# limix/CellRegMap

Hardware: AMD Instinct MI355X
Metric: variant-tests/sec (interaction test) (higher is better)
Workload: dtype f64

## Files before the change

### cellregmap_amd/csrc/api_core.hip

```cpp
#include <dlfcn.h>

#include <algorithm>
#include <atomic>
#include <cstdarg>
#include <mutex>

#include <map>

#include "crm_internal.h"
#include "eigh.h"

namespace crm {

static thread_local std::string g_error;

void set_error(const char* fmt, ...) {
    char buf[1024];
    va_list ap;
    va_start(ap, fmt);
    vsnprintf(buf, sizeof buf, fmt, ap);
    va_end(ap);
    g_error = buf;
}

// ... 131 lines not shown
    if (ptr) check_redzone(ptr, bytes);
    if (ptr) (void)hipFree(ptr);
    g_live_bytes -= (long)bytes;
    ptr = nullptr;
    bytes = 0;
    serial = 0;
}

int upload_padded(hipStream_t st, double* dst, long ld_dst, long rows_pad, const double* src,
                  long ld_src, long rows, long cols) {
    CRM_HIP(hipMemsetAsync(dst, 0, sizeof(double) * rows_pad * ld_dst, st));
    if (rows > 0 && cols > 0)
        CRM_HIP(hipMemcpy2DAsync(dst, ld_dst * sizeof(double), src, ld_src * sizeof(double),
                                 cols * sizeof(double), rows, hipMemcpyHostToDevice, st));
    return CRM_OK;
}

}

using namespace crm;

extern "C" {

const char* crm_last_error(void) { return last_error_text(); }
const char* crm_version(void) { return "0.6.0"; }

int crm_ctx_create(int device, crm_ctx** out) {
    return crm::guarded("crm_ctx_create", [&]() -> int {
    if (!out) return CRM_ERR_ARG;
    *out = nullptr;
    int count = 0;
    CRM_HIP(hipGetDeviceCount(&count));
    if (device < 0 || device >= count) {
        set_error("crm_ctx_create: device %d not present (%d visible)", device, count);
        return CRM_ERR_ARG;
    }
    CRM_HIP(hipSetDevice(device));
    crm_ctx* c = new crm_ctx();
    c->device = device;
    if (const char* e = getenv("CRM_KIN_ROUTE")) c->kin_route = std::max(0, std::min(2, atoi(e)));
    CRM_HIP(hipStreamCreateWithFlags(&c->stream, hipStreamNonBlocking));
    CRM_HIP(hipStreamCreateWithFlags(&c->upload_stream, hipStreamNonBlocking));
    CRM_HIP(hipEventCreate(&c->ev0));
    CRM_HIP(hipEventCreate(&c->ev1));
    int prio_least = 0, prio_greatest = 0;
    CRM_HIP(hipDeviceGetStreamPriorityRange(&prio_least, &prio_greatest));
    CRM_HIP(hipStreamCreateWithPriority(&c->side_stream, hipStreamNonBlocking, prio_least));
    for (hipEvent_t* e : {&c->ev_fork, &c->ev_side, &c->ev_main, &c->ev_fits}) CRM_HIP(hipEventCreateWithFlags(e, hipEventDisableTiming));
    {
        std::lock_guard<std::mutex> lock(g_ctx_mutex);
        g_contexts.push_back(c);
    }
    *out = c;
    return CRM_OK;
    });
}

int crm_ctx_trim(crm_ctx* c) {
    return crm::guarded_on("crm_ctx_trim", c, [&]() -> int {
    if (!c) return CRM_ERR_ARG;
    CRM_HIP(hipSetDevice(c->device));
    CRM_HIP(hipStreamSynchronize(c->stream));
    if (c->side_stream) CRM_HIP(hipStreamSynchronize(c->side_stream));
    std::lock_guard<std::mutex> lock(g_ctx_mutex);
    (void)trim_context(c);
    return CRM_OK;
    });
}

void crm_ctx_destroy(crm_ctx* c) {
    try {
    if (!c) return;
    (void)hipSetDevice(c->device);
    (void)hipStreamSynchronize(c->stream);
    if (c->side_stream) (void)hipStreamSynchronize(c->side_stream);
    {
        std::lock_guard<std::mutex> lock(g_ctx_mutex);
        g_contexts.erase(std::remove(g_contexts.begin(), g_contexts.end(), c), g_contexts.end());
        delete c->eigh_ws;
        c->eigh_ws = nullptr;
    }
    c->replay_clear();
    for (auto* b : c->all_bufs()) b->release();
    for (auto& e : c->timed) {
        (void)hipEventDestroy(e.first);
        (void)hipEventDestroy(e.second);
    }
    (void)hipEventDestroy(c->ev0);
    (void)hipEventDestroy(c->ev1);
    for (hipEvent_t e : {c->ev_fork, c->ev_side, c->ev_main, c->ev_fits})
        if (e) (void)hipEventDestroy(e);
    if (c->side_stream) (void)hipStreamDestroy(c->side_stream);
    (void)hipStreamDestroy(c->stream);
    if (c->upload_stream) (void)hipStreamDestroy(c->upload_stream);
    if (c->sync_timeouts_host) (void)hipHostFree(c->sync_timeouts_host);
    delete c;
    } catch (...) {
    }
}

int crm_ctx_synchronize(crm_ctx* c) {
    return crm::guarded_on("crm_ctx_synchronize", c, [&]() -> int {
    if (!c) return CRM_ERR_ARG;
    CRM_HIP(hipSetDevice(c->device));
    CRM_HIP(hipStreamSynchronize(c->stream));
    if (c->side_stream) CRM_HIP(hipStreamSynchronize(c->side_stream));
    return CRM_OK;
    });
}

int crm_set_block_variants(crm_ctx* c, int variants) {
    return crm::guarded_on("crm_set_block_variants", c, [&]() -> int {
    if (!c || variants < 0) return CRM_ERR_ARG;
    c->block_variants = variants == 0 ? 0 : (int)round_up(variants, 128);
    return CRM_OK;
    });
}

int crm_set_null_fit_polish(crm_ctx* c, int on) {
    return crm::guarded_on("crm_set_null_fit_polish", c, [&]() -> int {
    if (!c) return CRM_ERR_ARG;
    c->polish = on != 0;
    return CRM_OK;
    });
}

int crm_set_progress_callback(crm_ctx* c, void (*callback)(long, long, void*), void* user) {
    return crm::guarded_on("crm_set_progress_callback", c, [&]() -> int {
    if (!c) return CRM_ERR_ARG;
    if (callback) c->progress[std::this_thread::get_id()] = crm_ctx::Progress{callback, user};
    else c->progress.erase(std::this_thread::get_id());
    return CRM_OK;
    });
}

int crm_set_fast_rotation(crm_ctx* c, int on) {
    return crm::guarded_on("crm_set_fast_rotation", c, [&]() -> int {
    if (!c) return CRM_ERR_ARG;
    c->fast_T = on != 0;
    return CRM_OK;
    });
}

extern "C++" {
namespace crm {
namespace {
struct FormSlot { const char* name; int value; bool set; };
FormSlot g_forms[] = {{"gram_staged", 0, false}, {"kr_no_tail", 0, false}, {"nullfit_per_wave", 0, false}, {"kin_fold", 0, false},
                      {"eigh_one_stage", 0, false}, {"nullfit_exact", 0, false}, {"donor_pairs", 0, false},
                      {"pairs_without_kinship_term", 0, false}, {"flat_kappa_milli", 0, false}, {"chase_abort", 0, false}, {"nullfit_one_per_wave", 0, false},
                      {"kin_diag", 0, false}, {"donor_pairs_rotate", 0, false}, {"rho0_positions", 0, false},
                      {"rotation_tails", 0, false}, {"woodbury_ytY", 0, false},
                      {"wb_block_order", 0, false}, {"block_fused", 0, false}, {"wb_gram_fused", 0, false},
                      {"gram_strips", 0, false}, {"side_stream", 0, false}, {"wb_gram_spread", 0, false}};
std::mutex g_forms_mu;
}
int form(const char* name, int otherwise) {
    std::lock_guard<std::mutex> lock(g_forms_mu);
    for (const FormSlot& f : g_forms)
        if (strcmp(f.name, name) == 0) return f.set ? f.value : otherwise;
    return otherwise;
}
}
}

int crm_test_set_form(const char* name, int value, int reset) {
    return crm::guarded("crm_test_set_form", [&]() -> int {
    if (!name) return CRM_ERR_ARG;
    std::lock_guard<std::mutex> lock(crm::g_forms_mu);
    for (crm::FormSlot& f : crm::g_forms)
        if (strcmp(f.name, name) == 0) {
            f.value = value;
            f.set = reset == 0;
            return CRM_OK;
        }
    crm::set_error("crm_test_set_form: no kernel form is called '%s'", name);
    return CRM_ERR_ARG;
    });
}

long crm_test_tail_launches(const crm_ctx* ctx) { return ctx ? ctx->tail_launches : -1; }

long crm_test_spectrum_tail_launches(const crm_ctx* ctx) { return ctx ? ctx->spectrum_tail_launches : -1; }

long crm_test_dense_repeats(const crm_ctx* ctx) { return ctx ? ctx->dense_repeats : -1; }

long crm_test_donor_pair_blocks(const crm_ctx* ctx) { return ctx ? ctx->donor_pair_blocks : -1; }

int crm_test_gram_dma_launches(const crm_ctx* ctx, long* launches) {
    return crm::guarded("crm_test_gram_dma_launches", [&]() -> int {
    if (!ctx || !launches) return CRM_ERR_ARG;
    *launches = ctx->gram_dma_launches;
    return CRM_OK;
    });
}
int crm_test_unrelated_donor_blocks(const crm_ctx* ctx, long* blocks) {
    return crm::guarded("crm_test_unrelated_donor_blocks", [&]() -> int {
    if (!ctx || !blocks) return CRM_ERR_ARG;
    *blocks = ctx->unrelated_donor_blocks;
    return CRM_OK;
    });
}

int crm_test_fused_blocks(const crm_ctx* ctx, long* blocks) {
    return crm::guarded("crm_test_fused_blocks", [&]() -> int {
    if (!ctx || !blocks) return CRM_ERR_ARG;
    *blocks = ctx->fused_blocks;
    return CRM_OK;
    });
}

int crm_test_wb_gram_fused_blocks(const crm_ctx* ctx, long* blocks) {
    return crm::guarded("crm_test_wb_gram_fused_blocks", [&]() -> int {
    if (!ctx || !blocks) return CRM_ERR_ARG;
    *blocks = ctx->wb_gram_fused_blocks;
    return CRM_OK;
    });
}

int crm_test_side_stream_blocks(const crm_ctx* ctx, long* blocks) {
    return crm::guarded("crm_test_side_stream_blocks", [&]() -> int {
    if (!ctx || !blocks) return CRM_ERR_ARG;
    *blocks = ctx->side_stream_blocks;
    return CRM_OK;
    });
}

int crm_test_rho0_position_blocks(const crm_ctx* ctx, long* blocks) {
    return crm::guarded("crm_test_rho0_position_blocks", [&]() -> int {
    if (!ctx || !blocks) return CRM_ERR_ARG;
    *blocks = ctx->rho0_position_blocks;
    return CRM_OK;
    });
}
int crm_test_rotation_tail_launches(const crm_ctx* ctx, long* launches) {
    return crm::guarded("crm_test_rotation_tail_launches", [&]() -> int {
    if (!ctx || !launches) return CRM_ERR_ARG;
    *launches = ctx->rotation_tail_launches;
    return CRM_OK;
    });
}

long crm_test_tests_without_pair(const crm_ctx* ctx) { return ctx ? ctx->tests_without_pair : -1; }

int crm_test_set_shared_h(crm_ctx* ctx, int mode) {
    return crm::guarded_on("crm_test_set_shared_h", ctx, [&]() -> int {
    if (!ctx) return CRM_ERR_ARG;
    ctx->tune.shared_h = mode < 0 ? -1 : (mode > 0 ? 1 : 0);
    return CRM_OK;
    });
}

int crm_kernel_timer_reset(crm_ctx* c) {
    return crm::guarded_on("crm_kernel_timer_reset", c, [&]() -> int {
    if (!c) return CRM_ERR_ARG;
    CRM_HIP(hipSetDevice(c->device));
    CRM_HIP(hipStreamSynchronize(c->stream));
    c->timed_used = 0;
    c->kr_flops = 0.0;
    c->timing = true;
    return CRM_OK;
    });
}

int crm_kernel_timer_stop(crm_ctx* c) {
    return crm::guarded_on("crm_kernel_timer_stop", c, [&]() -> int {
    if (!c) return CRM_ERR_ARG;
    c->timing = false;
    return CRM_OK;
    });
}

int crm_kernel_timer_read(crm_ctx* c, double* kr_ms, long* kr_launches, double* kr_flops,
                          double* total_ms) {
    return crm::guarded_on("crm_kernel_timer_read", c, [&]() -> int {
    if (!c) return CRM_ERR_ARG;
    CRM_HIP(hipSetDevice(c->device));
    CRM_HIP(hipStreamSynchronize(c->stream));
    double ms = 0.0;
    for (size_t i = 0; i < c->timed_used; i++) {
        float t = 0.f;
        CRM_HIP(hipEventElapsedTime(&t, c->timed[i].first, c->timed[i].second));
        ms += t;
    }
    if (kr_ms) *kr_ms = ms;
    if (kr_launches) *kr_launches = (long)c->timed_used;
    if (kr_flops) *kr_flops = c->kr_flops;
    if (total_ms) *total_ms = 0.0;
    return CRM_OK;
    });
}

int crm_test_set_contraction(crm_ctx* c, int tile_width, int lds_dma) {
    return crm::guarded_on("crm_test_set_contraction", c, [&]() -> int {
    if (!c || (tile_width != 0 && tile_width != 64 && tile_width != 128 && tile_width != 160)) return CRM_ERR_ARG;
    c->tune.bn = tile_width;
    c->tune.glds = lds_dma ? 1 : 0;
    return CRM_OK;
    });
}

long crm_test_sync_fallbacks(const crm_ctx* c) { return c ? c->sync_fallbacks : -1; }
long crm_test_overruns(void) { return crm::overruns_detected(); }
long crm_test_live_device_bytes(void) { return crm::live_device_bytes(); }

int crm_test_set_kinship_route(crm_ctx* c, int on) {
    return crm::guarded_on("crm_test_set_kinship_route", c, [&]() -> int {
// ... 254 lines not shown
```

### cellregmap_amd/csrc/nullfit.hip

```cpp
#include "crm_internal.h"
#include "delta_search.h"
#include "wave_ops.h"
#include <type_traits>

namespace crm {

namespace {

template <int N, int FROM>
__device__ inline void butterfly_sums(double (&v)[N]) {
    double t[N];
    if constexpr (FROM >= 32) {
#pragma unroll
        for (int i = 0; i < N; i++) t[i] = __shfl_xor(v[i], 32, 64);
#pragma unroll
        for (int i = 0; i < N; i++) v[i] += t[i];
#pragma unroll
        for (int i = 0; i < N; i++) t[i] = lane_xor_swizzle(v[i], 16);
#pragma unroll
        for (int i = 0; i < N; i++) v[i] += t[i];
    }
#pragma unroll
    for (int i = 0; i < N; i++) t[i] = lane_xor_swizzle(v[i], 8);
#pragma unroll
    for (int i = 0; i < N; i++) v[i] += t[i];
#pragma unroll
    for (int i = 0; i < N; i++) t[i] = lane_xor_swizzle(v[i], 4);
#pragma unroll
    for (int i = 0; i < N; i++) v[i] += t[i];
#pragma unroll
    for (int i = 0; i < N; i++) t[i] = lane_xor_quad(v[i], 2);
#pragma unroll
    for (int i = 0; i < N; i++) v[i] += t[i];
#pragma unroll
    for (int i = 0; i < N; i++) t[i] = lane_xor_quad(v[i], 1);
#pragma unroll
    for (int i = 0; i < N; i++) v[i] += t[i];
}

__device__ inline double fast_rcp(double D) {
    double x = __builtin_amdgcn_rcp(D);
    double e = fma(-D, x, 1.0);
    x = fma(x, e, x);
    e = fma(-D, x, 1.0);
    return fma(x, e, x);
}

struct LogProduct {
    double mant = 1.0;
    int expo = 0;
    __device__ inline void mul(double D) {
        mant *= __builtin_amdgcn_frexp_mant(D);
        expo += __builtin_amdgcn_frexp_exp(D);
    }
    __device__ inline void renorm() {
        expo += __builtin_amdgcn_frexp_exp(mant);
        mant = __builtin_amdgcn_frexp_mant(mant);
    }
    __device__ inline double log_value() const { return log(mant) + (double)expo * 0.6931471805599453; }
};

__host__ __device__ constexpr int pair_index(int u, int v, int U) {
    return u * U - u * (u - 1) / 2 + (v - u);
}

template <int P>
__device__ inline bool cholesky(double (&A)[P][P], double& logdet) {
    logdet = 0.0;
#pragma unroll
    for (int j = 0; j < P; j++) {
        double d = A[j][j];
#pragma unroll
        for (int k = 0; k < j; k++) d -= A[j][k] * A[j][k];
        if (!(d > 0.0)) return false;
        const double l = sqrt(d);
        A[j][j] = l;
        logdet += 2.0 * log(l);
#pragma unroll
        for (int i = j + 1; i < P; i++) {
            double s = A[i][j];
#pragma unroll
            for (int k = 0; k < j; k++) s -= A[i][k] * A[j][k];
            A[i][j] = s / l;
        }
    }
    return true;
}

template <int P>
__device__ inline bool cholesky_pivots(double (&A)[P][P], double (&piv)[P]) {
#pragma unroll
    for (int j = 0; j < P; j++) {
        double d = A[j][j];
#pragma unroll
        for (int k = 0; k < j; k++) d -= A[j][k] * A[j][k];
        if (!(d > 0.0)) return false;
        const double l = sqrt(d);
        A[j][j] = l;
        piv[j] = l;
#pragma unroll
        for (int i = j + 1; i < P; i++) {
            double s = A[i][j];
#pragma unroll
            for (int k = 0; k < j; k++) s -= A[i][k] * A[j][k];
            A[i][j] = s / l;
        }
    }
    return true;
}

template <int P>
__device__ inline void cholesky_solve(const double (&L)[P][P], double (&b)[P]) {
#pragma unroll
    for (int i = 0; i < P; i++) {
        double s = b[i];
#pragma unroll
        for (int k = 0; k < i; k++) s -= L[i][k] * b[k];
        b[i] = s / L[i][i];
    }
#pragma unroll
    for (int i = P - 1; i >= 0; i--) {
        double s = b[i];
#pragma unroll
        for (int k = i + 1; k < P; k++) s -= L[k][i] * b[k];
        b[i] = s / L[i][i];
    }
}

template <int U>
__device__ __noinline__ double objective_noise_bound(const double (&bb)[U], const double (&sd)[U], const double (&pl)[U * (U + 1) / 2],
                                                     double inv_d, double rss, double df, double lsum, double n_minus_r, double log_delta,
                                                     double n, double log_s, double logdetXX, double logdetH, double p_eff) {
    double mag = 0.0;
#pragma unroll
    for (int u = 0; u < U; u++)
#pragma unroll
        for (int v = u; v < U; v++) {
            const double spec = sqrt(fabs(sd[u] * sd[v]));
            const double m_uv = spec + pl[pair_index(u, v, U)] * inv_d;
            mag += (u == v ? 1.0 : 2.0) * bb[u] * bb[v] * m_uv;
        }
    const double logs = fabs(lsum) + fabs(n_minus_r) * fabs(log_delta) + n * fabs(log_s) + df * (LOG2PI + 1.0) + fabs(logdetXX) +
                        fabs(logdetH) + p_eff * fabs(log_s);
    return 0.5 * (df * mag / fabs(rss) + logs);
}

template <int C, bool SH, bool EX, bool TR, int G = 1>
__device__ __forceinline__ void nullfit_fit(const NullFitArgs& a, const int b, const int w, const int lane,
                                            const double* sW, const double* sy, const double* sS, const int sld) {
    static_assert(G == 1 || (G == 4 && C == 1 && !EX), "four fits per wavefront: one covariate column, default arithmetic");
    const int sub = G == 1 ? lane : (lane & 15);
    constexpr int P = C + 1;
    constexpr int U = C + 2;
    constexpr int NP = U * (U + 1) / 2;
    const NullFitRho R = a.rho[w];
    const double* __restrict__ tg = R.T + (long)b * R.ldT;
    const int r = R.r;
    const double n = (double)a.n;

    double uv[NP];
#pragma unroll
    for (int i = 0; i < C; i++) {
#pragma unroll
        for (int j = i; j < C; j++) uv[pair_index(i, j, U)] = a.WW[i * C + j];
        uv[pair_index(i, C, U)] = a.gW[(long)b * a.ld_gW + i];
        uv[pair_index(i, C + 1, U)] = a.Wy[i];
    }
    uv[pair_index(C, C, U)] = a.gg[b];
    uv[pair_index(C, C + 1, U)] = a.gy[b];
    uv[pair_index(C + 1, C + 1, U)] = a.yy;

    bool use_g = true;
    double logdetXX = 0.0;
    {
        double A[P][P];
#pragma unroll
        for (int i = 0; i < P; i++)
#pragma unroll
            for (int j = 0; j <= i; j++) A[i][j] = uv[pair_index(j, i, U)];
        double ld = 0.0;
        bool ok = true;
#pragma unroll
        for (int j = 0; j < P; j++) {
            double d = A[j][j];
#pragma unroll
            for (int k = 0; k < j; k++) d -= A[j][k] * A[j][k];
            if (j == P - 1) {
                if (a.g_drop ? a.g_drop[b] != 0 : !(d > 1e-12 * A[j][j])) {
                    use_g = false;
                    break;
                }
                if (!(d > 0.0)) {
                    ok = false;
                    break;
                }
            } else if (!(d > 0.0)) {
                ok = false;
                break;
            }
            const double l = sqrt(d);
            A[j][j] = l;
            ld += 2.0 * log(l);
#pragma unroll
            for (int i = j + 1; i < P; i++) {
                double s = A[i][j];
#pragma unroll
                for (int k = 0; k < j; k++) s -= A[i][k] * A[j][k];
                A[i][j] = s / l;
            }
        }
        logdetXX = ok ? ld : NAN;
    }
    const double p_eff = use_g ? (double)P : (double)C;
    const double df = a.restricted ? n - p_eff : n;

    auto spectrum_pass = [&](double delta, bool weighted, double (&S)[NP], double& lsum,
                             bool grad, double (&S2)[NP], double& lsum2) {
#pragma unroll
        for (int i = 0; i < NP; i++) { S[i] = 0.0; S2[i] = 0.0; }
        lsum = 0.0;
        lsum2 = 0.0;
        LogProduct lp;
        int trips = 0;
        const double omd = 1.0 - delta;
        constexpr int UNR = C <= 2 ? 4 : 2;
        auto trip = [&](const int j0, auto full_tag) {
            constexpr bool FULL = decltype(full_tag)::value;
            double t[UNR][U], s0[UNR];
            bool ok[UNR];
#pragma unroll
            for (int q = 0; q < UNR; q++) {
                const int j = j0 + 64 * q;
                ok[q] = FULL || j < r;
                const int jj = ok[q] ? j : r - 1;
#pragma unroll
                for (int i = 0; i < C; i++) t[q][i] = SH ? sW[i * sld + jj] : R.tW[(long)i * R.ldW + jj];
                t[q][C] = tg[jj];
                t[q][C + 1] = SH ? sy[jj] : R.ty[jj];
                s0[q] = weighted ? (SH ? sS[jj] : R.S0[jj]) : 0.0;
            }
#pragma unroll
            for (int q = 0; q < UNR; q++) {
                double wgt = ok[q] ? 1.0 : 0.0, wgt2 = 0.0;
                if (weighted) {
                    const double D = ok[q] ? omd * s0[q] + delta : 1.0;
                    const double inv = EX ? 1.0 / D : fast_rcp(D);
                    wgt = ok[q] ? inv : 0.0;
                    if (EX) lsum += log(D);
                    else lp.mul(D);
                    if (grad) {
                        const double oms = 1.0 - s0[q];
                        lsum2 += ok[q] ? oms * inv : 0.0;
                        wgt2 = ok[q] ? oms * inv * inv : 0.0;
                    }
                }
#pragma unroll
                for (int u = 0; u < U; u++) {
                    const double tw = t[q][u] * wgt;
                    const double tw2 = t[q][u] * wgt2;
#pragma unroll
                    for (int v = u; v < U; v++) {
                        S[pair_index(u, v, U)] += tw * t[q][v];
                        if (grad) S2[pair_index(u, v, U)] += tw2 * t[q][v];
                    }
                }
            }
        };
        for (int j0 = lane; j0 < r; j0 += 64 * UNR) {
            if (j0 - lane + 64 * UNR - 1 < r) trip(j0, std::true_type{});
            else trip(j0, std::false_type{});
            if (!EX && weighted && (++trips & 127) == 0) lp.renorm();
        }
        {
            double red[NP + 1];
#pragma unroll
            for (int i = 0; i < NP; i++) red[i] = S[i];
            red[NP] = weighted ? (EX ? lsum : lp.log_value()) : 0.0;
            butterfly_sums<NP + 1, 32>(red);
#pragma unroll
            for (int i = 0; i < NP; i++) S[i] = red[i];
            if (weighted) lsum = red[NP];
        }
        if (grad) {
            double red[NP + 1];
#pragma unroll
            for (int i = 0; i < NP; i++) red[i] = S2[i];
            red[NP] = lsum2;
            butterfly_sums<NP + 1, 32>(red);
#pragma unroll
            for (int i = 0; i < NP; i++) S2[i] = red[i];
            lsum2 = red[NP];
        }
    };

    auto spectrum_pass4 = [&](double delta, bool weighted, double (&S)[NP], double& lsum) {
        double Sq[4][NP];
        LogProduct lpq[4];
#pragma unroll
        for (int q = 0; q < 4; q++)
#pragma unroll
            for (int i = 0; i < NP; i++) Sq[q][i] = 0.0;
        const double omd = 1.0 - delta;
        int trips[4];
#pragma unroll
        for (int q = 0; q < 4; q++) trips[q] = sub + 16 * q < r ? (r - (sub + 16 * q) + 255) / 256 : 0;
        const int t_all = (r + 255) / 256;
        for (int t = 0; t < t_all; t++) {
            const bool full = 256 * t + 255 < r;
#pragma unroll
            for (int q = 0; q < 4; q++) {
                if (!full && t >= trips[q]) continue;
                double tv[4][U], s0[4];
                bool ok[4];
#pragma unroll
                for (int k = 0; k < 4; k++) {
                    const int j = sub + 16 * q + 64 * (4 * t + k);
                    ok[k] = full || j < r;
                    const int jj = ok[k] ? j : r - 1;
#pragma unroll
                    for (int i = 0; i < C; i++) tv[k][i] = SH ? sW[i * sld + jj] : R.tW[(long)i * R.ldW + jj];
                    tv[k][C] = tg[jj];
                    tv[k][C + 1] = SH ? sy[jj] : R.ty[jj];
                    s0[k] = weighted ? (SH ? sS[jj] : R.S0[jj]) : 0.0;
                }
#pragma unroll
                for (int k = 0; k < 4; k++) {
                    double wgt = ok[k] ? 1.0 : 0.0;
                    if (weighted) {
                        const double D = ok[k] ? omd * s0[k] + delta : 1.0;
                        const double inv = fast_rcp(D);
                        wgt = ok[k] ? inv : 0.0;
                        lpq[q].mul(D);
                    }
#pragma unroll
                    for (int u = 0; u < U; u++) {
                        const double tw = tv[k][u] * wgt;
#pragma unroll
                        for (int v = u; v < U; v++) Sq[q][pair_index(u, v, U)] += tw * tv[k][v];
                    }
                }
                if (weighted && ((t + 1) & 127) == 0) lpq[q].renorm();
            }
        }
        double red[NP + 1];
#pragma unroll
        for (int i = 0; i < NP; i++) red[i] = (Sq[0][i] + Sq[2][i]) + (Sq[1][i] + Sq[3][i]);
        red[NP] = weighted ? (lpq[0].log_value() + lpq[2].log_value()) + (lpq[1].log_value() + lpq[3].log_value()) : 0.0;
        butterfly_sums<NP + 1, 8>(red);
#pragma unroll
        for (int i = 0; i < NP; i++) S[i] = red[i];
        lsum = weighted ? red[NP] : 0.0;
    };

    double tt[NP];
    {
        double dummy, dummy2, unused[NP];
        if constexpr (G == 1) spectrum_pass(1.0, false, tt, dummy, false, unused, dummy2);
        else spectrum_pass4(1.0, false, tt, dummy);
    }

    double cur_delta = 0.5, cur_scale = 1.0, cur_lml = -INFINITY;
    int nfev = 0;
    double memo_f[2] = {0.0, 0.0}, memo_scale[2] = {0.0, 0.0}, memo_lml[2] = {0.0, 0.0}, memo_noise[2] = {NAN, NAN};
    bool memo_set[2] = {false, false};
    bool last_clamped = false;
    bool want_noise = false;
    double cur_noise = NAN;
    auto f = [&](double x) -> double {
        nfev++;
        const double delta = logistic_clamped(x);
        const int clamp = delta == 1.0 - EPS_TINY ? 1 : (delta == EPS_TINY ? 0 : -1);
        last_clamped = clamp >= 0;
        if (clamp >= 0 && memo_set[clamp]) {
            cur_delta = delta;
            cur_scale = memo_scale[clamp];
            cur_lml = memo_lml[clamp];
            cur_noise = memo_noise[clamp];
            return memo_f[clamp];
        }
        auto remember = [&](double value) -> double {
            if (clamp >= 0) {
                memo_set[clamp] = true;
                memo_f[clamp] = value;
                memo_scale[clamp] = cur_scale;
                memo_lml[clamp] = cur_lml;
                memo_noise[clamp] = cur_noise;
            }
            return value;
        };
        double S[NP], lsum;
        if constexpr (G == 1) {
            double unused[NP], unused2;
            spectrum_pass(delta, true, S, lsum, false, unused, unused2);
        } else {
            spectrum_pass4(delta, true, S, lsum);
        }
        const double inv_d = 1.0 / delta;
        double K[NP];
#pragma unroll
        for (int i = 0; i < NP; i++) K[i] = S[i] + (uv[i] - tt[i]) * inv_d;
        double A[P][P], rhs[P], xky[P];
#pragma unroll
        for (int i = 0; i < P; i++) {
#pragma unroll
            for (int j = 0; j <= i; j++) A[i][j] = K[pair_index(j, i, U)];
            rhs[i] = K[pair_index(i, C + 1, U)];
        }
        if (!use_g) {
#pragma unroll
            for (int j = 0; j < C; j++) A[C][j] = 0.0;
            A[C][C] = 1.0;
            rhs[C] = 0.0;
        }
#pragma unroll
        for (int i = 0; i < P; i++) xky[i] = rhs[i];
        double piv[P];
        double val;
        if (!cholesky_pivots<P>(A, piv)) {
            cur_delta = delta;
            cur_scale = NAN;
            cur_lml = NAN;
            return remember(INFINITY);
        }
        cholesky_solve<P>(A, rhs);
        double rss = K[pair_index(C + 1, C + 1, U)];
#pragma unroll
        for (int i = 0; i < P; i++) rss -= xky[i] * rhs[i];
        const double s = fmax(rss / df, EPS_SMALL);
        double larg = 1.0;
        larg = sub == 0 ? delta : larg;
#pragma unroll
        for (int j = 0; j < P; j++) larg = sub == 1 + j ? piv[j] : larg;
        larg = sub == P + 1 ? s : larg;
        const double lres = log(larg);
        auto from_sub = [&](int k) -> double {
            if constexpr (G == 1) return read_lane(lres, k);
            else return __shfl(lres, (lane & 48) + k, 64);
        };
        const double log_delta = from_sub(0), log_s = from_sub(P + 1);
        double logdetH = 0.0;
#pragma unroll
        for (int j = 0; j < P; j++) logdetH += 2.0 * from_sub(1 + j);
        const double logdetK = lsum + (n - (double)r) * log_delta;
        val = -0.5 * (df * LOG2PI + df + n * log_s + logdetK);
        if (a.restricted) val += 0.5 * (logdetXX - (logdetH - p_eff * log_s));
        cur_delta = delta;
        cur_scale = s;
        cur_lml = val;
        if constexpr (TR) {
            if (want_noise || clamp >= 0) {
                double bb[U], sd[U], pl[NP];
#pragma unroll
                for (int i = 0; i < P; i++) bb[i] = fabs(rhs[i]);
                bb[P] = 1.0;
#pragma unroll
                for (int u = 0; u < U; u++) sd[u] = S[pair_index(u, u, U)];
#pragma unroll
                for (int i = 0; i < NP; i++) pl[i] = fabs(uv[i]) + fabs(tt[i]);
                cur_noise = objective_noise_bound<U>(bb, sd, pl, inv_d, rss, df, lsum, (n - (double)r), log_delta, n, log_s, logdetXX,
                                                     logdetH, p_eff);
            }
        }
        return remember(-val);
    };

    auto g = [&](double x) -> double {
        const double delta = logistic_clamped(x);
        if (delta <= EPS_TINY || delta >= 1.0 - EPS_TINY) return 0.0;
        double S[NP], S2[NP], lsum, lsum2;
        spectrum_pass(delta, true, S, lsum, true, S2, lsum2);
        const double inv_d = 1.0 / delta, inv_d2 = inv_d * inv_d;
        double K[NP], dK[NP];
#pragma unroll
        for (int i = 0; i < NP; i++) {
            const double cpl = uv[i] - tt[i];
            K[i] = S[i] + cpl * inv_d;
            dK[i] = -S2[i] - cpl * inv_d2;
        }
        const double dlogdet = lsum2 + (n - (double)r) * inv_d;
        double A[P][P], dA[P][P], b[P], db[P], beta[P];
#pragma unroll
        for (int i = 0; i < P; i++) {
#pragma unroll
            for (int j = 0; j < P; j++) {
                const int pi = i <= j ? pair_index(i, j, U) : pair_index(j, i, U);
                A[i][j] = K[pi];
                dA[i][j] = dK[pi];
            }
            b[i] = K[pair_index(i, C + 1, U)];
            db[i] = dK[pair_index(i, C + 1, U)];
        }
        if (!use_g) {
#pragma unroll
            for (int j = 0; j < P; j++) {
                A[C][j] = 0.0; A[j][C] = 0.0;
                dA[C][j] = 0.0; dA[j][C] = 0.0;
            }
            A[C][C] = 1.0;
            b[C] = 0.0;
            db[C] = 0.0;
        }
        double ld;
        if (!cholesky<P>(A, ld)) return NAN;
#pragma unroll
        for (int i = 0; i < P; i++) beta[i] = b[i];
        cholesky_solve<P>(A, beta);
        double Rv = K[pair_index(C + 1, C + 1, U)];
        double dR = dK[pair_index(C + 1, C + 1, U)];
#pragma unroll
        for (int i = 0; i < P; i++) {
            Rv -= b[i] * beta[i];
            dR -= 2.0 * db[i] * beta[i];
#pragma unroll
            for (int j = 0; j < P; j++) dR += beta[i] * dA[i][j] * beta[j];
        }
        double d = df * dR / Rv + dlogdet;
        if (a.restricted) {
            double tr = 0.0;
#pragma unroll
            for (int j = 0; j < P; j++) {
                double col[P];
#pragma unroll
                for (int i = 0; i < P; i++) col[i] = dA[i][j];
                cholesky_solve<P>(A, col);
                tr += col[j];
            }
            d += tr;
        }
        return 0.5 * d * delta * (1.0 - delta);
    };

    if (a.probe) {
        (void)f(a.probe_x);
        if (sub == 0) {
            NullFitTrial t;
            t.lml = cur_lml; t.delta = cur_delta; t.scale = cur_scale; t.use_g = use_g ? 1 : 0; t.nfev = nfev;
            t.margin = NAN; t.noise = NAN; t.curv = NAN;
            a.trial[(long)b * a.nrho + w] = t;
        }
        return;
    }
    {
        struct Objective {
            decltype(f)& fn;
            const bool& at_clamp;
            __device__ inline double operator()(double x) { return fn(x); }
            __device__ inline bool clamped() const { return at_clamp; }
        } objective{f, last_clamped};
        BrentTrace trace;
        double bf0;
        double bx0 = brent_search<TR>(objective, trace, bf0);
        if constexpr (G == 1) if (a.polish) {
            const double xs = bx0, fs = bf0;
            double xa = xs, ga = g(xa);
            if (isfinite(ga) && ga != 0.0) {
                double xb = ga > 0.0 ? xa - 1e-4 : xa + 1e-4;
                double gb = g(xb);
                bool reject = false;
                for (int it = 0; it < 8; it++) {
                    if (!isfinite(gb) || gb == ga) break;
                    const double xn = xb - gb * (xb - xa) / (gb - ga);
                    if (!isfinite(xn) || fabs(xn - xs) > 1e-2) { reject = true; break; }
                    const double step = fabs(xn - xb);
                    xa = xb; ga = gb;
                    xb = xn;
                    gb = g(xb);
                    if (gb == 0.0 || step <= 1e-12 * (1.0 + fabs(xn))) break;
                }
                if (!reject && isfinite(gb)) {
                    const double fb = f(xb);
                    if (fb <= fs + 1e-9 * fabs(fs)) bx0 = xb;
                }
            }
        }
        double f_up = NAN, f_dn = NAN;
        if constexpr (TR) {
            const double tolx = 1e-6 * fabs(bx0) + 1e-6;
            f_up = f(bx0 + tolx);
            f_dn = f(bx0 - tolx);
        }
        want_noise = true;
        const double f_stop = f(bx0);
        if (sub == 0) {
            NullFitTrial t;
            t.lml = cur_lml;
            t.delta = cur_delta;
            t.scale = cur_scale;
            t.use_g = use_g ? 1 : 0;
            t.nfev = nfev;
            if constexpr (TR) {
                t.margin = fmin(trace.cmp, trace.sign);
                t.curv = 0.5 * (f_up + f_dn) - f_stop;
                t.noise = cur_noise;
            } else {
                (void)f_stop;
                t.margin = NAN; t.curv = NAN; t.noise = NAN;
            }
            a.trial[(long)b * a.nrho + w] = t;
        }
    }
}

template <int C, bool EX, bool TR>
#ifdef CRM_NULLFIT_WAVES
__attribute__((amdgpu_waves_per_eu(CRM_NULLFIT_WAVES, CRM_NULLFIT_WAVES)))
#endif
__global__ __launch_bounds__(64) void nullfit_kernel(NullFitArgs a) {
    nullfit_fit<C, false, EX, TR, 1>(a, (int)blockIdx.x, (int)blockIdx.y, (int)threadIdx.x, nullptr, nullptr, nullptr, 0);
}

constexpr int nf_shared_waves(int G) { return G == 1 ? 12 : 8; }
template <int C, bool EX, bool TR, int G>
__global__ __launch_bounds__(64 * nf_shared_waves(G)) void nullfit_shared_kernel(NullFitArgs a, int variants, int sld,
                                                                             unsigned* __restrict__ queue) {
    extern __shared__ double nf_sm[];
    __shared__ int any_left;
    double* const sW = nf_sm;
    double* const sy = nf_sm + C * sld;
    double* const sS = sy + sld;
    const int tid = threadIdx.x, lane = tid & 63;
    const int w0 = (int)(blockIdx.x % (unsigned)a.nrho);
    for (int pass = 0; pass < a.nrho; pass++) {
        const int w = (w0 + pass) % a.nrho;
        if (tid == 0)
            any_left = __hip_atomic_load(&queue[w], __ATOMIC_RELAXED, __HIP_MEMORY_SCOPE_AGENT) < (unsigned)variants;
        __syncthreads();
        const bool any = any_left != 0;
        __syncthreads();
        if (!any) continue;
        const NullFitRho R = a.rho[w];
        for (int j = tid; j < R.r; j += 64 * nf_shared_waves(G)) {
#pragma unroll
            for (int i = 0; i < C; i++) sW[i * sld + j] = R.tW[(long)i * R.ldW + j];
            sy[j] = R.ty[j];
            sS[j] = R.S0[j];
        }
        __syncthreads();
        for (;;) {
            const unsigned ticket = __hip_atomic_fetch_add(&queue[w], lane == 0 ? (unsigned)G : 0u, __ATOMIC_RELAXED,
                                                           __HIP_MEMORY_SCOPE_AGENT);
            const unsigned b0 = (unsigned)__builtin_amdgcn_readfirstlane((int)ticket);
            if (b0 >= (unsigned)variants) break;
            if constexpr (G == 1) {
                nullfit_fit<C, true, EX, TR, 1>(a, (int)b0, w, lane, sW, sy, sS, sld);
            } else {
                const unsigned b = b0 + (unsigned)(lane >> 4);
                if (b < (unsigned)variants) nullfit_fit<C, true, EX, TR, G>(a, (int)b, w, lane, sW, sy, sS, sld);
            }
        }
        __syncthreads();
    }
}

__global__ void select_rho_kernel(const NullFitTrial* __restrict__ trial, int nrho, int variants,
                                  NullFitOut* __restrict__ out) {
    const int b = blockIdx.x * blockDim.x + threadIdx.x;
    if (b >= variants) return;
    double best = -INFINITY;
    int bi = -1;
    bool fitted = true;
    for (int i = 0; i < nrho; i++) {
        const NullFitTrial t = trial[(long)b * nrho + i];
        if (t.nfev <= 0) fitted = false;
        if (t.lml > best) {
            best = t.lml;
            bi = i;
        }
    }
    NullFitOut o;
    o.use_g = trial[(long)b * nrho].use_g;
    o.decision = NAN; o.rho_decision = NAN; o.margin = NAN; o.noise = NAN; o.gap = NAN; o.curv = NAN;
    if (!fitted) {
        o.rho_index = -1;
        o.lml = NAN; o.delta = NAN; o.scale = NAN; o.v0 = NAN; o.v1 = NAN;
    } else if (bi < 0) {
        o.rho_index = 0;
        o.lml = NAN; o.delta = NAN; o.scale = NAN; o.v0 = NAN; o.v1 = NAN;
    } else {
        const NullFitTrial t = trial[(long)b * nrho + bi];
        o.rho_index = bi;
        o.lml = best;
        o.delta = t.delta;
        o.scale = t.scale;
        o.v0 = t.scale * (1.0 - t.delta);
        o.v1 = t.scale * t.delta;
        constexpr double ROUNDING = 1.1102230246251565e-16;
        o.margin = t.margin;
        o.noise = t.noise;
        o.curv = t.curv;
        o.decision = t.margin / (ROUNDING * t.noise);
        double gap = INFINITY, rdec = INFINITY;
        for (int i = 0; i < nrho; i++) {
            if (i == bi) continue;
            const NullFitTrial q = trial[(long)b * nrho + i];
            const double g = best - q.lml;
            gap = fmin(gap, g);
            rdec = fmin(rdec, g / (ROUNDING * (t.noise + q.noise)));
        }
        o.gap = gap;
        o.rho_decision = rdec;
    }
    out[b] = o;
}

}

template <int C>
static void launch_c(hipStream_t st, const NullFitArgs& a, int variants) {
    if (a.exact) hipLaunchKernelGGL((nullfit_kernel<C, true, false>), dim3(variants, a.nrho), dim3(64), 0, st, a);
    else if (a.track) hipLaunchKernelGGL((nullfit_kernel<C, false, true>), dim3(variants, a.nrho), dim3(64), 0, st, a);
    else hipLaunchKernelGGL((nullfit_kernel<C, false, false>), dim3(variants, a.nrho), dim3(64), 0, st, a);
}

int launch_nullfit(hipStream_t st, const NullFitArgs& a, int variants, bool force_wide, unsigned* queue) {
    if (variants <= 0) return CRM_OK;
    if (a.nrho < 1 || a.nrho > CRM_MAX_RHO) {
        set_error("null fit: %d grid points (supported 1..%d)", a.nrho, CRM_MAX_RHO);
        return CRM_ERR_UNSUPPORTED;
    }
    CRM_HIP(hipMemsetAsync(a.trial, 0xFF, sizeof(NullFitTrial) * (size_t)variants * a.nrho, st));
    int rmax = 1;
    for (int i = 0; i < a.nrho; i++) rmax = std::max(rmax, a.rho[i].r);
    const int sld = (rmax + 63) / 64 * 64;
    const size_t shared_lds = sizeof(double) * 3 * (size_t)sld;
    if (queue && !force_wide && a.c == 1 && variants >= 1024 && shared_lds <= 144 * 1024 && !form("nullfit_per_wave", 0)) {
        int cus = 256, dev = 0;
        CRM_HIP(hipGetDevice(&dev));
        CRM_HIP(hipDeviceGetAttribute(&cus, hipDeviceAttributeMultiprocessorCount, dev));
        CRM_HIP(hipMemsetAsync(queue, 0, sizeof(unsigned) * CRM_MAX_RHO, st));
        const bool four = !a.exact && !a.polish && rmax <= 2048 && !form("nullfit_one_per_wave", 0);
#define CRM_NF_SHARED(EXv, TRv, Gv)                                                                                        \
    do {                                                                                                                   \
        const void* fn = reinterpret_cast<const void*>(&nullfit_shared_kernel<1, EXv, TRv, Gv>);                           \
        if (shared_lds > 60 * 1024)                                                                                        \
            CRM_HIP(hipFuncSetAttribute(fn, hipFuncAttributeMaxDynamicSharedMemorySize, (int)shared_lds));                 \
        hipLaunchKernelGGL((nullfit_shared_kernel<1, EXv, TRv, Gv>), dim3(cus), dim3(64 * nf_shared_waves(Gv)), shared_lds, st, a, \
                           variants, sld, queue);                                                                          \
    } while (0)
        if (a.exact) CRM_NF_SHARED(true, false, 1);
        else if (a.track && four) CRM_NF_SHARED(false, true, 4);
        else if (a.track) CRM_NF_SHARED(false, true, 1);
        else if (four) CRM_NF_SHARED(false, false, 4);
        else CRM_NF_SHARED(false, false, 1);
#undef CRM_NF_SHARED
    } else if (a.c > CRM_MAX_COV_WIDE) {
        CRM_TRY(launch_nullfit_xwide(st, a, variants));
    } else if (force_wide || a.c > CRM_MAX_COV) {
        CRM_TRY(launch_nullfit_wide(st, a, variants));
    } else
    switch (a.c) {
        case 1: launch_c<1>(st, a, variants); break;
        case 2: launch_c<2>(st, a, variants); break;
        case 3: launch_c<3>(st, a, variants); break;
        case 4: launch_c<4>(st, a, variants); break;
        case 5: launch_c<5>(st, a, variants); break;
        case 6: launch_c<6>(st, a, variants); break;
        case 7: launch_c<7>(st, a, variants); break;
        case 8: launch_c<8>(st, a, variants); break;
        default:
            set_error("null fit: %d covariate columns (supported 1..%d)", a.c, CRM_MAX_COV);
            return CRM_ERR_UNSUPPORTED;
    }
    CRM_HIP(hipGetLastError());
    hipLaunchKernelGGL(select_rho_kernel, dim3((variants + 127) / 128), dim3(128), 0, st, a.trial, a.nrho,
                       variants, a.out);
    CRM_HIP(hipGetLastError());
    return CRM_OK;
}

}
```

Baseline: 85190.

## Share variant-independent spectrum sums across null fits and reuse the opening evaluations

In the shared-LDS null-fit kernel, the variant-independent weighted Gram sums of covariates and phenotype are computed once per rho grid point for delta=1 and the two opening deltas and stored in LDS. Each variant then runs one fused pass that computes only its genotype cross terms for all three deltas. The opening objective evaluations at x=0 and x=1 are served from a per-wave memo, and the final objective evaluation is skipped when the best point was already evaluated. This trades extra LDS, register pressure and a serial per-block precompute for fewer per-variant spectrum passes.

Result: no change. 86020, median of 6 (+1.0%).

```diff
diff --git a/cellregmap_amd/csrc/api_core.hip b/cellregmap_amd/csrc/api_core.hip
--- a/cellregmap_amd/csrc/api_core.hip
+++ b/cellregmap_amd/csrc/api_core.hip
@@ -307,7 +307,8 @@
                       {"kin_diag", 0, false}, {"donor_pairs_rotate", 0, false}, {"rho0_positions", 0, false},
                       {"rotation_tails", 0, false}, {"woodbury_ytY", 0, false},
                       {"wb_block_order", 0, false}, {"block_fused", 0, false}, {"wb_gram_fused", 0, false},
-                      {"gram_strips", 0, false}, {"side_stream", 0, false}, {"wb_gram_spread", 0, false}};
+                      {"gram_strips", 0, false}, {"side_stream", 0, false}, {"wb_gram_spread", 0, false},
+                      {"nullfit_opening", 0, false}};
 std::mutex g_forms_mu;
 }
 int form(const char* name, int otherwise) {
diff --git a/cellregmap_amd/csrc/nullfit.hip b/cellregmap_amd/csrc/nullfit.hip
--- a/cellregmap_amd/csrc/nullfit.hip
+++ b/cellregmap_amd/csrc/nullfit.hip
@@ -64,6 +64,9 @@
     return u * U - u * (u - 1) / 2 + (v - u);
 }
 
+constexpr int nf_grid_sums(int C) { return (C + 1) * (C + 2) / 2; }
+constexpr int NF_MEMO = 10;
+
 template <int P>
 __device__ inline bool cholesky(double (&A)[P][P], double& logdet) {
     logdet = 0.0;
@@ -145,9 +148,97 @@
     return 0.5 * (df * mag / fabs(rss) + logs);
 }
 
+template <int C, bool GP>
+__device__ __forceinline__ void opening_pass(const double* tg, const double* sW, const double* sy, const double* sS, const int sld,
+                                             const int r, const int lane, const double d0, const double d1,
+                                             double (&Sk)[3][GP ? (C + 1) * (C + 2) / 2 : C + 2], double (&lsum)[3]) {
+    constexpr int V = C + 1;
+    constexpr int NS = GP ? V * (V + 1) / 2 : C + 2;
+    constexpr int UNR = C <= 2 ? 4 : 2;
+#pragma unroll
+    for (int k = 0; k < 3; k++)
+#pragma unroll
+        for (int i = 0; i < NS; i++) Sk[k][i] = 0.0;
+    LogProduct lp[2];
+    int trips = 0;
+    const double omd0 = 1.0 - d0, omd1 = 1.0 - d1;
+    auto trip = [&](const int j0, auto full_tag) {
+        constexpr bool FULL = decltype(full_tag)::value;
+        double t[UNR][V], g[UNR], s0[UNR];
+        bool ok[UNR];
+#pragma unroll
+        for (int q = 0; q < UNR; q++) {
+            const int j = j0 + 64 * q;
+            ok[q] = FULL || j < r;
+            const int jj = ok[q] ? j : r - 1;
+#pragma unroll
+            for (int i = 0; i < C; i++) t[q][i] = sW[i * sld + jj];
+            t[q][C] = sy[jj];
+            g[q] = GP ? 0.0 : tg[jj];
+            s0[q] = sS[jj];
+        }
+#pragma unroll
+        for (int q = 0; q < UNR; q++) {
+            const double D0 = ok[q] ? fma(omd0, s0[q], d0) : 1.0;
+            const double D1 = ok[q] ? fma(omd1, s0[q], d1) : 1.0;
+            const double inv0 = fast_rcp(D0), inv1 = fast_rcp(D1);
+            const double wgt[3] = {ok[q] ? 1.0 : 0.0, ok[q] ? inv0 : 0.0, ok[q] ? inv1 : 0.0};
+            if constexpr (GP) {
+                lp[0].mul(D0);
+                lp[1].mul(D1);
+            }
+#pragma unroll
+            for (int k = 0; k < 3; k++) {
+                if constexpr (GP) {
+                    int i = 0;
+#pragma unroll
+                    for (int u = 0; u < V; u++) {
+                        const double tw = t[q][u] * wgt[k];
+#pragma unroll
+                        for (int v = u; v < V; v++, i++) Sk[k][i] = fma(tw, t[q][v], Sk[k][i]);
+                    }
+                } else {
+#pragma unroll
+                    for (int i = 0; i < C; i++) Sk[k][i] = fma(t[q][i] * wgt[k], g[q], Sk[k][i]);
+                    const double gw = g[q] * wgt[k];
+                    Sk[k][C] = fma(gw, g[q], Sk[k][C]);
+                    Sk[k][C + 1] = fma(gw, t[q][C], Sk[k][C + 1]);
+                }
+            }
+        }
+    };
+    for (int j0 = lane; j0 < r; j0 += 64 * UNR) {
+        if (j0 - lane + 64 * UNR - 1 < r) trip(j0, std::true_type{});
+        else trip(j0, std::false_type{});
+        if (GP && (++trips & 127) == 0) {
+            lp[0].renorm();
+            lp[1].renorm();
+        }
+    }
+    constexpr int NR = 3 * NS + (GP ? 2 : 0);
+    double red[NR];
+#pragma unroll
+    for (int k = 0; k < 3; k++)
+#pragma unroll
+        for (int i = 0; i < NS; i++) red[k * NS + i] = Sk[k][i];
+    if constexpr (GP) {
+        red[3 * NS] = lp[0].log_value();
+        red[3 * NS + 1] = lp[1].log_value();
+    }
+    butterfly_sums<NR, 32>(red);
+#pragma unroll
+    for (int k = 0; k < 3; k++)
+#pragma unroll
+        for (int i = 0; i < NS; i++) Sk[k][i] = red[k * NS + i];
+    lsum[0] = 0.0;
+    lsum[1] = GP ? red[NR - 2] : 0.0;
+    lsum[2] = GP ? red[NR - 1] : 0.0;
+}
+
 template <int C, bool SH, bool EX, bool TR, int G = 1>
 __device__ __forceinline__ void nullfit_fit(const NullFitArgs& a, const int b, const int w, const int lane,
-                                            const double* sW, const double* sy, const double* sS, const int sld) {
+                                            const double* sW, const double* sy, const double* sS, const int sld,
+                                            const bool opening, const double* sc, double* memo) {
     static_assert(G == 1 || (G == 4 && C == 1 && !EX), "four fits per wavefront: one covariate column, default arithmetic");
     const int sub = G == 1 ? lane : (lane & 15);
     constexpr int P = C + 1;
@@ -352,20 +443,135 @@
         lsum = weighted ? red[NP] : 0.0;
     };
 
-    double tt[NP];
-    {
-        double dummy, dummy2, unused[NP];
-        if constexpr (G == 1) spectrum_pass(1.0, false, tt, dummy, false, unused, dummy2);
-        else spectrum_pass4(1.0, false, tt, dummy);
-    }
-
     double cur_delta = 0.5, cur_scale = 1.0, cur_lml = -INFINITY;
     int nfev = 0;
+    double tt[NP];
+    constexpr bool KEEP_BEST = !TR && !EX;
+    bool opened = false;
+    if constexpr (KEEP_BEST) {
+        memo[0] = NAN;
+        memo[3] = INFINITY;
+    }
+    auto note_best = [&](double x, double value) {
+        if constexpr (KEEP_BEST) {
+            if (value <= memo[3]) {
+                memo[0] = x;
+                memo[1] = cur_scale;
+                memo[2] = cur_lml;
+                memo[3] = value;
+            }
+        }
+    };
     double memo_f[2] = {0.0, 0.0}, memo_scale[2] = {0.0, 0.0}, memo_lml[2] = {0.0, 0.0}, memo_noise[2] = {NAN, NAN};
     bool memo_set[2] = {false, false};
     bool last_clamped = false;
     bool want_noise = false;
     double cur_noise = NAN;
+    auto objective_of_sums = [&](const double delta, const double (&S)[NP], const double lsum, const bool noise_now) -> double {
+        const double inv_d = 1.0 / delta;
+        double K[NP];
+#pragma unroll
+        for (int i = 0; i < NP; i++) K[i] = S[i] + (uv[i] - tt[i]) * inv_d;
+        double A[P][P], rhs[P], xky[P];
+#pragma unroll
+        for (int i = 0; i < P; i++) {
+#pragma unroll
+            for (int j = 0; j <= i; j++) A[i][j] = K[pair_index(j, i, U)];
+            rhs[i] = K[pair_index(i, C + 1, U)];
+        }
+        if (!use_g) {
+#pragma unroll
+            for (int j = 0; j < C; j++) A[C][j] = 0.0;
+            A[C][C] = 1.0;
+            rhs[C] = 0.0;
+        }
+#pragma unroll
+        for (int i = 0; i < P; i++) xky[i] = rhs[i];
+        double piv[P];
+        double val;
+        if (!cholesky_pivots<P>(A, piv)) {
+            cur_delta = delta;
+            cur_scale = NAN;
+            cur_lml = NAN;
+            return INFINITY;
+        }
+        cholesky_solve<P>(A, rhs);
+        double rss = K[pair_index(C + 1, C + 1, U)];
+#pragma unroll
+        for (int i = 0; i < P; i++) rss -= xky[i] * rhs[i];
+        const double s = fmax(rss / df, EPS_SMALL);
+        double larg = 1.0;
+        larg = sub == 0 ? delta : larg;
+#pragma unroll
+        for (int j = 0; j < P; j++) larg = sub == 1 + j ? piv[j] : larg;
+        larg = sub == P + 1 ? s : larg;
+        const double lres = log(larg);
+        auto from_sub = [&](int k) -> double {
+            if constexpr (G == 1) return read_lane(lres, k);
+            else return __shfl(lres, (lane & 48) + k, 64);
+        };
+        const double log_delta = from_sub(0), log_s = from_sub(P + 1);
+        double logdetH = 0.0;
+#pragma unroll
+        for (int j = 0; j < P; j++) logdetH += 2.0 * from_sub(1 + j);
+        const double logdetK = lsum + (n - (double)r) * log_delta;
+        val = -0.5 * (df * LOG2PI + df + n * log_s + logdetK);
+        if (a.restricted) val += 0.5 * (logdetXX - (logdetH - p_eff * log_s));
+        cur_delta = delta;
+        cur_scale = s;
+        cur_lml = val;
+        if constexpr (TR) {
+            if (noise_now) {
+                double bb[U], sd[U], pl[NP];
+#pragma unroll
+                for (int i = 0; i < P; i++) bb[i] = fabs(rhs[i]);
+                bb[P] = 1.0;
+#pragma unroll
+                for (int u = 0; u < U; u++) sd[u] = S[pair_index(u, u, U)];
+#pragma unroll
+                for (int i = 0; i < NP; i++) pl[i] = fabs(uv[i]) + fabs(tt[i]);
+                cur_noise = objective_noise_bound<U>(bb, sd, pl, inv_d, rss, df, lsum, (n - (double)r), log_delta, n, log_s, logdetXX,
+                                                     logdetH, p_eff);
+            }
+        }
+        return -val;
+    };
+
+    if constexpr (SH && G == 1 && !EX) {
+        if (opening && !a.probe) {
+            constexpr int SCS = nf_grid_sums(C) + 2;
+            const double d0 = sc[SCS + SCS - 1], d1 = sc[2 * SCS + SCS - 1];
+            double Sg[3][U], unused[3];
+            opening_pass<C, false>(tg, sW, sy, sS, sld, r, lane, d0, d1, Sg, unused);
+            auto sums_of = [&](const int k, double (&S)[NP]) {
+#pragma unroll
+                for (int u = 0; u < U; u++)
+#pragma unroll
+                    for (int v = u; v < U; v++) {
+                        const int i = pair_index(u, v, U);
+                        S[i] = v == C ? Sg[k][u]
+                                      : (u == C ? Sg[k][v] : sc[k * SCS + pair_index(u < C ? u : u - 1, v < C ? v : v - 1, C + 1)]);
+                    }
+            };
+            sums_of(0, tt);
+#pragma unroll 1
+            for (int k = 1; k <= 2; k++) {
+                double S[NP];
+                sums_of(k, S);
+                const double value = objective_of_sums(k == 1 ? d0 : d1, S, sc[k * SCS + SCS - 2], false);
+                memo[1 + 3 * k] = value;
+                memo[2 + 3 * k] = cur_scale;
+                memo[3 + 3 * k] = cur_lml;
+            }
+            opened = true;
+        }
+    }
+    if (!opened) {
+        double dummy, dummy2, unused[NP];
+        if constexpr (G == 1) spectrum_pass(1.0, false, tt, dummy, false, unused, dummy2);
+        else spectrum_pass4(1.0, false, tt, dummy);
+    }
+
     auto f = [&](double x) -> double {
         nfev++;
         const double delta = logistic_clamped(x);
@@ -376,92 +582,35 @@
             cur_scale = memo_scale[clamp];
             cur_lml = memo_lml[clamp];
             cur_noise = memo_noise[clamp];
+            note_best(x, memo_f[clamp]);
             return memo_f[clamp];
         }
-        auto remember = [&](double value) -> double {
-            if (clamp >= 0) {
-                memo_set[clamp] = true;
-                memo_f[clamp] = value;
-                memo_scale[clamp] = cur_scale;
-                memo_lml[clamp] = cur_lml;
-                memo_noise[clamp] = cur_noise;
-            }
-            return value;
-        };
-        double S[NP], lsum;
-        if constexpr (G == 1) {
-            double unused[NP], unused2;
-            spectrum_pass(delta, true, S, lsum, false, unused, unused2);
+        double value;
+        if (opened && !want_noise && (x == 0.0 || x == 1.0)) {
+            const int at = x == 0.0 ? 4 : 7;
+            cur_delta = delta;
+            value = memo[at];
+            cur_scale = memo[at + 1];
+            cur_lml = memo[at + 2];
         } else {
-            spectrum_pass4(delta, true, S, lsum);
-        }
-        const double inv_d = 1.0 / delta;
-        double K[NP];
-#pragma unroll
-        for (int i = 0; i < NP; i++) K[i] = S[i] + (uv[i] - tt[i]) * inv_d;
-        double A[P][P], rhs[P], xky[P];
-#pragma unroll
-        for (int i = 0; i < P; i++) {
-#pragma unroll
-            for (int j = 0; j <= i; j++) A[i][j] = K[pair_index(j, i, U)];
-            rhs[i] = K[pair_index(i, C + 1, U)];
-        }
-        if (!use_g) {
-#pragma unroll
-            for (int j = 0; j < C; j++) A[C][j] = 0.0;
-            A[C][C] = 1.0;
-            rhs[C] = 0.0;
-        }
-#pragma unroll
-        for (int i = 0; i < P; i++) xky[i] = rhs[i];
-        double piv[P];
-        double val;
-        if (!cholesky_pivots<P>(A, piv)) {
-            cur_delta = delta;
-            cur_scale = NAN;
-            cur_lml = NAN;
-            return remember(INFINITY);
-        }
-        cholesky_solve<P>(A, rhs);
-        double rss = K[pair_index(C + 1, C + 1, U)];
-#pragma unroll
-        for (int i = 0; i < P; i++) rss -= xky[i] * rhs[i];
-        const double s = fmax(rss / df, EPS_SMALL);
-        double larg = 1.0;
-        larg = sub == 0 ? delta : larg;
-#pragma unroll
-        for (int j = 0; j < P; j++) larg = sub == 1 + j ? piv[j] : larg;
-        larg = sub == P + 1 ? s : larg;
-        const double lres = log(larg);
-        auto from_sub = [&](int k) -> double {
-            if constexpr (G == 1) return read_lane(lres, k);
-            else return __shfl(lres, (lane & 48) + k, 64);
-        };
-        const double log_delta = from_sub(0), log_s = from_sub(P + 1);
-        double logdetH = 0.0;
-#pragma unroll
-        for (int j = 0; j < P; j++) logdetH += 2.0 * from_sub(1 + j);
-        const double logdetK = lsum + (n - (double)r) * log_delta;
-        val = -0.5 * (df * LOG2PI + df + n * log_s + logdetK);
-        if (a.restricted) val += 0.5 * (logdetXX - (logdetH - p_eff * log_s));
-        cur_delta = delta;
-        cur_scale = s;
-        cur_lml = val;
-        if constexpr (TR) {
-            if (want_noise || clamp >= 0) {
-                double bb[U], sd[U], pl[NP];
-#pragma unroll
-                for (int i = 0; i < P; i++) bb[i] = fabs(rhs[i]);
-                bb[P] = 1.0;
-#pragma unroll
-                for (int u = 0; u < U; u++) sd[u] = S[pair_index(u, u, U)];
-#pragma unroll
-                for (int i = 0; i < NP; i++) pl[i] = fabs(uv[i]) + fabs(tt[i]);
-                cur_noise = objective_noise_bound<U>(bb, sd, pl, inv_d, rss, df, lsum, (n - (double)r), log_delta, n, log_s, logdetXX,
-                                                     logdetH, p_eff);
-            }
-        }
-        return remember(-val);
+            double S[NP], lsum;
+            if constexpr (G == 1) {
+                double unused[NP], unused2;
+                spectrum_pass(delta, true, S, lsum, false, unused, unused2);
+            } else {
+                spectrum_pass4(delta, true, S, lsum);
+            }
+            value = objective_of_sums(delta, S, lsum, want_noise || clamp >= 0);
+        }
+        if (clamp >= 0) {
+            memo_set[clamp] = true;
+            memo_f[clamp] = value;
+            memo_scale[clamp] = cur_scale;
+            memo_lml[clamp] = cur_lml;
+            memo_noise[clamp] = cur_noise;
+        }
+        note_best(x, value);
+        return value;
     };
 
     auto g = [&](double x) -> double {
@@ -580,7 +729,18 @@
             f_dn = f(bx0 - tolx);
         }
         want_noise = true;
-        const double f_stop = f(bx0);
+        double f_stop;
+        bool from_memo = false;
+        if constexpr (KEEP_BEST) from_memo = opening && memo[0] == bx0;
+        if (from_memo) {
+            nfev++;
+            cur_delta = logistic_clamped(bx0);
+            cur_scale = memo[1];
+            cur_lml = memo[2];
+            f_stop = memo[3];
+        } else {
+            f_stop = f(bx0);
+        }
         if (sub == 0) {
             NullFitTrial t;
             t.lml = cur_lml;
@@ -605,19 +765,23 @@
 #ifdef CRM_NULLFIT_WAVES
 __attribute__((amdgpu_waves_per_eu(CRM_NULLFIT_WAVES, CRM_NULLFIT_WAVES)))
 #endif
-__global__ __launch_bounds__(64) void nullfit_kernel(NullFitArgs a) {
-    nullfit_fit<C, false, EX, TR, 1>(a, (int)blockIdx.x, (int)blockIdx.y, (int)threadIdx.x, nullptr, nullptr, nullptr, 0);
+__global__ __launch_bounds__(64) void nullfit_kernel(NullFitArgs a, int opening) {
+    __shared__ double memo[4];
+    nullfit_fit<C, false, EX, TR, 1>(a, (int)blockIdx.x, (int)blockIdx.y, (int)threadIdx.x, nullptr, nullptr, nullptr, 0, opening != 0,
+                                     nullptr, memo);
 }
 
 constexpr int nf_shared_waves(int G) { return G == 1 ? 12 : 8; }
 template <int C, bool EX, bool TR, int G>
 __global__ __launch_bounds__(64 * nf_shared_waves(G)) void nullfit_shared_kernel(NullFitArgs a, int variants, int sld,
-                                                                             unsigned* __restrict__ queue) {
+                                                                             unsigned* __restrict__ queue, int opening) {
     extern __shared__ double nf_sm[];
     __shared__ int any_left;
     double* const sW = nf_sm;
     double* const sy = nf_sm + C * sld;
     double* const sS = sy + sld;
+    double* const sc = sS + sld;
+    double* const memo = sc + 3 * (nf_grid_sums(C) + 2) + NF_MEMO * (G == 1 ? 4 * (threadIdx.x >> 6) : threadIdx.x >> 4);
     const int tid = threadIdx.x, lane = tid & 63;
     const int w0 = (int)(blockIdx.x % (unsigned)a.nrho);
     for (int pass = 0; pass < a.nrho; pass++) {
@@ -636,16 +800,36 @@
             sS[j] = R.S0[j];
         }
         __syncthreads();
+        if constexpr (G == 1 && !EX) {
+            if (opening) {
+                constexpr int NG = nf_grid_sums(C);
+                if (tid < 64) {
+                    double Sk[3][NG], lsum[3];
+                    const double dk[3] = {1.0, logistic_clamped(0.0), logistic_clamped(1.0)};
+                    opening_pass<C, true>(nullptr, sW, sy, sS, sld, R.r, lane, dk[1], dk[2], Sk, lsum);
+                    if (lane == 0) {
+#pragma unroll
+                        for (int k = 0; k < 3; k++) {
+#pragma unroll
+                            for (int i = 0; i < NG; i++) sc[k * (NG + 2) + i] = Sk[k][i];
+                            sc[k * (NG + 2) + NG] = lsum[k];
+                            sc[k * (NG + 2) + NG + 1] = dk[k];
+                        }
+                    }
+                }
+                __syncthreads();
+            }
+        }
         for (;;) {
             const unsigned ticket = __hip_atomic_fetch_add(&queue[w], lane == 0 ? (unsigned)G : 0u, __ATOMIC_RELAXED,
                                                            __HIP_MEMORY_SCOPE_AGENT);
             const unsigned b0 = (unsigned)__builtin_amdgcn_readfirstlane((int)ticket);
             if (b0 >= (unsigned)variants) break;
             if constexpr (G == 1) {
-                nullfit_fit<C, true, EX, TR, 1>(a, (int)b0, w, lane, sW, sy, sS, sld);
+                nullfit_fit<C, true, EX, TR, 1>(a, (int)b0, w, lane, sW, sy, sS, sld, opening != 0, sc, memo);
             } else {
                 const unsigned b = b0 + (unsigned)(lane >> 4);
-                if (b < (unsigned)variants) nullfit_fit<C, true, EX, TR, G>(a, (int)b, w, lane, sW, sy, sS, sld);
+                if (b < (unsigned)variants) nullfit_fit<C, true, EX, TR, G>(a, (int)b, w, lane, sW, sy, sS, sld, opening != 0, sc, memo);
             }
         }
         __syncthreads();
@@ -706,10 +890,10 @@
 }
 
 template <int C>
-static void launch_c(hipStream_t st, const NullFitArgs& a, int variants) {
-    if (a.exact) hipLaunchKernelGGL((nullfit_kernel<C, true, false>), dim3(variants, a.nrho), dim3(64), 0, st, a);
-    else if (a.track) hipLaunchKernelGGL((nullfit_kernel<C, false, true>), dim3(variants, a.nrho), dim3(64), 0, st, a);
-    else hipLaunchKernelGGL((nullfit_kernel<C, false, false>), dim3(variants, a.nrho), dim3(64), 0, st, a);
+static void launch_c(hipStream_t st, const NullFitArgs& a, int variants, int opening) {
+    if (a.exact) hipLaunchKernelGGL((nullfit_kernel<C, true, false>), dim3(variants, a.nrho), dim3(64), 0, st, a, opening);
+    else if (a.track) hipLaunchKernelGGL((nullfit_kernel<C, false, true>), dim3(variants, a.nrho), dim3(64), 0, st, a, opening);
+    else hipLaunchKernelGGL((nullfit_kernel<C, false, false>), dim3(variants, a.nrho), dim3(64), 0, st, a, opening);
 }
 
 int launch_nullfit(hipStream_t st, const NullFitArgs& a, int variants, bool force_wide, unsigned* queue) {
@@ -723,19 +907,21 @@
     for (int i = 0; i < a.nrho; i++) rmax = std::max(rmax, a.rho[i].r);
     const int sld = (rmax + 63) / 64 * 64;
     const size_t shared_lds = sizeof(double) * 3 * (size_t)sld;
+    const int opening = form("nullfit_opening", 1);
     if (queue && !force_wide && a.c == 1 && variants >= 1024 && shared_lds <= 144 * 1024 && !form("nullfit_per_wave", 0)) {
         int cus = 256, dev = 0;
         CRM_HIP(hipGetDevice(&dev));
         CRM_HIP(hipDeviceGetAttribute(&cus, hipDeviceAttributeMultiprocessorCount, dev));
         CRM_HIP(hipMemsetAsync(queue, 0, sizeof(unsigned) * CRM_MAX_RHO, st));
         const bool four = !a.exact && !a.polish && rmax <= 2048 && !form("nullfit_one_per_wave", 0);
+        const size_t lds = shared_lds + sizeof(double) * (3 * (nf_grid_sums(1) + 2) + NF_MEMO * 4 * nf_shared_waves(1));
 #define CRM_NF_SHARED(EXv, TRv, Gv)                                                                                        \
     do {                                                                                                                   \
         const void* fn = reinterpret_cast<const void*>(&nullfit_shared_kernel<1, EXv, TRv, Gv>);                           \
-        if (shared_lds > 60 * 1024)                                                                                        \
-            CRM_HIP(hipFuncSetAttribute(fn, hipFuncAttributeMaxDynamicSharedMemorySize, (int)shared_lds));                 \
-        hipLaunchKernelGGL((nullfit_shared_kernel<1, EXv, TRv, Gv>), dim3(cus), dim3(64 * nf_shared_waves(Gv)), shared_lds, st, a, \
-                           variants, sld, queue);                                                                          \
+        if (lds > 60 * 1024)                                                                                               \
+            CRM_HIP(hipFuncSetAttribute(fn, hipFuncAttributeMaxDynamicSharedMemorySize, (int)lds));                        \
+        hipLaunchKernelGGL((nullfit_shared_kernel<1, EXv, TRv, Gv>), dim3(cus), dim3(64 * nf_shared_waves(Gv)), lds, st, a, \
+                           variants, sld, queue, opening);                                                                 \
     } while (0)
         if (a.exact) CRM_NF_SHARED(true, false, 1);
         else if (a.track && four) CRM_NF_SHARED(false, true, 4);
@@ -749,14 +935,14 @@
         CRM_TRY(launch_nullfit_wide(st, a, variants));
     } else
     switch (a.c) {
-        case 1: launch_c<1>(st, a, variants); break;
-        case 2: launch_c<2>(st, a, variants); break;
-        case 3: launch_c<3>(st, a, variants); break;
-        case 4: launch_c<4>(st, a, variants); break;
-        case 5: launch_c<5>(st, a, variants); break;
-        case 6: launch_c<6>(st, a, variants); break;
-        case 7: launch_c<7>(st, a, variants); break;
-        case 8: launch_c<8>(st, a, variants); break;
+        case 1: launch_c<1>(st, a, variants, opening); break;
+        case 2: launch_c<2>(st, a, variants, opening); break;
+        case 3: launch_c<3>(st, a, variants, opening); break;
+        case 4: launch_c<4>(st, a, variants, opening); break;
+        case 5: launch_c<5>(st, a, variants, opening); break;
+        case 6: launch_c<6>(st, a, variants, opening); break;
+        case 7: launch_c<7>(st, a, variants, opening); break;
+        case 8: launch_c<8>(st, a, variants, opening); break;
         default:
             set_error("null fit: %d covariate columns (supported 1..%d)", a.c, CRM_MAX_COV);
             return CRM_ERR_UNSUPPORTED;
```
